# edenartlab/sd-lora-trainer

Measured on AMD Instinct MI355X. Metric: training images/sec, SDXL 1024px rank-16 LoRA, 1/2/4/8 GPU (job-parallel), higher is better.
Workload: dtype bf16

## Files before the change

### include/sdlt_kernels.h

```cpp
#ifndef SDLT_KERNELS_H
#define SDLT_KERNELS_H
#include <stdint.h>
#ifdef __cplusplus
extern "C" {
#endif

const char* sdlt_last_error(void);
int sdlt_abi_version(void);
int sdlt_struct_size(int which);

typedef struct sdlt_gemm_batch_item {
  const void* X; const void* W;
  const void* Adown; const void* Bup; void* T_out;
  void* C; void* Ct;
  const float* bias;
  const float* col_scale;
} sdlt_gemm_batch_item;

typedef struct sdlt_gemm_params {
  const void* X; int64_t ldx;
  const void* W; int64_t ldw;
  int32_t M, N, K;
  const void* X2; int64_t ldx2;
  const void* W2; int64_t ldw2;
// ... 58 lines not shown
  const void* Q; int64_t ldq;
  float* out;
  int32_t M, Cw, R, Rp;
  int32_t rank_major;
  int32_t accumulate;
  int32_t conv, Hin, Win, Cin, Hout, Wout, stride;
  const void* zero;
  int32_t first_block;
  int32_t pad_;
} sdlt_lora_grad_desc;
int sdlt_lora_grad_grouped(const sdlt_lora_grad_desc* descs_dev, const int32_t* block_desc_dev,
                           int32_t n_blocks, int32_t Rp, int32_t mfma, void* stream);
int32_t sdlt_lora_grad_block_cols(void);
int sdlt_lora_grad_wide(const sdlt_lora_grad_desc* descs_dev, const int32_t* block_desc_dev,
                        int32_t n_blocks, int32_t Rp, int32_t mfma, void* stream);

typedef struct sdlt_attn_params {
  const void* Q; int64_t ldq;
  const void* K; int64_t ldk;
  const void* V; int64_t ldv;
  const void* Kt; int64_t ldkt;
  const void* Vt; int64_t ldvt;
  const void* Qt; int64_t ldqt;
  const void* dOt; int64_t lddot;
  void* O; int64_t ldo;
  float* L;
  const void* dO; int64_t lddo;
  float* D;
  void* dQ; int64_t lddq;
  void* dK; int64_t lddk;
// ... 490 lines not shown
```

### sd-lora-trainer_amd/_lib.py

```python
import ctypes as C
import os

import torch

_HERE = os.path.dirname(os.path.abspath(__file__))
LIB_PATH = os.environ.get("SDLT_KERNEL_LIB") or os.path.join(_HERE, "libsdlt_kernels.so")

i32, i64, f32, vp = C.c_int32, C.c_int64, C.c_float, C.c_void_p


class GemmParams(C.Structure):
    _fields_ = [
        ("X", vp), ("ldx", i64), ("W", vp), ("ldw", i64),
        ("M", i32), ("N", i32), ("K", i32),
        ("X2", vp), ("ldx2", i64), ("W2", vp), ("ldw2", i64),
        ("K2", i32), ("mode", i32),
        ("Hin", i32), ("Win", i32), ("Cin", i32), ("Hout", i32), ("Wout", i32),
        ("stride", i32), ("ups", i32), ("flip", i32), ("tr", i32),
        ("zero", vp),
        ("Adown", vp), ("ld_adown", i64), ("Bup", vp), ("ld_bup", i64),
        ("T_out", vp), ("ld_t", i64),
        ("lora_R", i32), ("lora_scale", f32), ("alpha", f32),
        ("bias", vp),
        ("rowbias", vp), ("ld_rowbias", i64), ("rows_per_batch", i32),
# ... 51 lines not shown
    _fields_ = [("dY", vp), ("lddy", i64), ("Y", vp), ("ldy", i64), ("bias", vp), ("mag", vp), ("scale", vp), ("gmag", vp), ("gB", vp),
                ("ws_off", i64), ("M", i32), ("N", i32), ("rank", i32), ("splits", i32), ("grad_scale", f32), ("accumulate", i32)]


class LoraGradDesc(C.Structure):
    _fields_ = [
        ("P", vp), ("ldp", i64), ("Q", vp), ("ldq", i64), ("out", vp),
        ("M", i32), ("Cw", i32), ("R", i32), ("Rp", i32),
        ("rank_major", i32), ("accumulate", i32),
        ("conv", i32), ("Hin", i32), ("Win", i32), ("Cin", i32), ("Hout", i32), ("Wout", i32), ("stride", i32),
        ("zero", vp),
        ("first_block", i32), ("pad_", i32),
    ]


class AttnParams(C.Structure):
    _fields_ = [
        ("Q", vp), ("ldq", i64), ("K", vp), ("ldk", i64), ("V", vp), ("ldv", i64),
        ("Kt", vp), ("ldkt", i64), ("Vt", vp), ("ldvt", i64), ("Qt", vp), ("ldqt", i64), ("dOt", vp), ("lddot", i64),
        ("O", vp), ("ldo", i64), ("L", vp),
        ("dO", vp), ("lddo", i64), ("D", vp),
        ("dQ", vp), ("lddq", i64), ("dK", vp), ("lddk", i64), ("dV", vp), ("lddv", i64),
        ("dK32", vp), ("dV32", vp), ("ld32", i64),
        ("B", i32), ("H", i32), ("Nq", i32), ("Nk", i32), ("Nqp", i32), ("Nkp", i32), ("d", i32),
        ("scale", f32), ("qsplit", i32), ("causal", i32), ("accumulate_dq", i32), ("accumulate_dk", i32), ("defer_splitsum", i32), ("d_ready", i32),
    ]


ATTN_ROUTES = ("FWD32", "FWD16_KS2", "FWD16", "BWD_CROSS_ROLES", "BWD_CROSS", "BWD_BOTH32", "BWD_BOTH16", "BWD_SPLIT")
ATTN_ROUTE_MASK = 0xF
# ... 132 lines not shown

class ShadowDesc(C.Structure):
    _fields_ = [("offset", i64), ("src_ld", i64), ("rows", i32), ("cols", i32), ("dst", vp), ("ld", i64), ("dstT", vp), ("ldT", i64)]


SYMBOLS = {
    "sdlt_last_error": (C.c_char_p, []),
    "sdlt_abi_version": (i32, []),
    "sdlt_struct_size": (i32, [i32]),
    "sdlt_add2d": (i32, [vp, i64, vp, i64, vp, i64, i32, i32, vp]),
    "sdlt_gemm_bf16": (i32, [C.POINTER(GemmParams), vp]),
    "sdlt_gemm_route": (i32, [C.POINTER(GemmParams), C.POINTER(GemmPlan)]),
    "sdlt_lora_grad_grouped": (i32, [vp, vp, i32, i32, i32, vp]),
    "sdlt_lora_grad_block_cols": (i32, []),
    "sdlt_lora_grad_wide": (i32, [vp, vp, i32, i32, i32, vp]),
    "sdlt_attn_fwd": (i32, [C.POINTER(AttnParams), vp]),
    "sdlt_attn_bwd": (i32, [C.POINTER(AttnParams), vp]),
    "sdlt_attn_route": (i32, [C.POINTER(AttnParams), i32]),
    "sdlt_attn_splitsum_batch": (i32, [vp, vp, vp, i32, vp]),
    "sdlt_groupnorm_ws_floats": (i32, [i32, i32, i32]),
    "sdlt_colsum_finish_batch": (i32, [vp, i32, i32, vp]),
    "sdlt_groupnorm_fwd": (i32, [C.POINTER(GroupNormParams), vp]),
    "sdlt_groupnorm_bwd": (i32, [C.POINTER(GroupNormParams), vp]),
    "sdlt_layernorm_fwd": (i32, [vp, i64, i32, i32, vp, vp, f32, vp, i64, vp, vp]),
    "sdlt_layernorm_bwd": (i32, [vp, i64, vp, i64, i32, i32, vp, vp, vp, i64, vp, i64, vp]),
    "sdlt_layernorm_bwd_y": (i32, [vp, i64, vp, i64, i32, i32, vp, vp, vp, vp, i64, vp, i64, vp, i64, vp]),
    "sdlt_ln_fold_adapters": (i32, [vp, i32, vp]),
    "sdlt_layernorm_bwd_slabs": (i32, [vp, i64, vp, i64, i32, i32, i32, vp, vp, vp, i64, vp, i64, vp]),
    "sdlt_geglu_fwd": (i32, [vp, i64, i32, i32, vp, i64, vp]),
    "sdlt_geglu_bwd": (i32, [vp, i64, vp, i64, i32, i32, vp, i64, vp]),
# ... 80 lines not shown
            "(hipcc --offload-arch=gfx950).  There is no CPU / PyTorch fallback for the training step.")
    lib = C.CDLL(LIB_PATH, mode=C.RTLD_GLOBAL)
    for name, (res, args) in SYMBOLS.items():
        try:
            fn = getattr(lib, name)
        except AttributeError as e:
            raise KernelLibraryError(f"{LIB_PATH} does not export {name}") from e
        fn.restype = res
        fn.argtypes = args
    for which, (name, size) in enumerate(struct_sizes()):
        if lib.sdlt_struct_size(which) != size:
            raise KernelLibraryError(f"struct layout mismatch for {name}: C {lib.sdlt_struct_size(which)} vs binding {size}")
    if C.sizeof(ResizeParams) != 48:
        raise KernelLibraryError(f"struct layout mismatch for ResizeParams: header 48 vs binding {C.sizeof(ResizeParams)}")
    for cls, size in ((HeatAccumParams, 152), (HeatOverlayParams, 80), (GemmPlan, 64), (SamplerDdParams, 128), (WindowParams, 64), (RegionParams, 64),
                      (GuidanceApgParams, 56), (GuidanceDynParams, 48)):
        if C.sizeof(cls) != size:
            raise KernelLibraryError(f"struct layout mismatch for {cls.__name__}: header {size} vs binding {C.sizeof(cls)}")
    _lib = lib
    return lib


def struct_sizes():
    mirrored = (GemmParams, LoraGradDesc, AttnParams, GroupNormParams, ShadowDesc, GemmBatchItem, DoraDesc, DoraWtDesc, DoraGradDesc, SplitsumDesc, StripParams,
                TaParams, LnSlabsParams, TaGroup)
    return [(c.__name__, C.sizeof(c)) for c in mirrored] + [("sdlt_affine_grad_item", 8 * 8), ("sdlt_wgrad_tr_item", 3 * 8), ("LnFoldDesc", C.sizeof(LnFoldDesc)), ("ColsumFinishDesc", C.sizeof(ColsumFinishDesc)),
                                                               ("WskGemmParams", C.sizeof(WskGemmParams)), ("MergeDesc", C.sizeof(MergeDesc)), ("SamplerParams", C.sizeof(SamplerParams)),
                                                               ("DeltaDesc", C.sizeof(DeltaDesc)), ("SamplerImgParams", C.sizeof(SamplerImgParams)),
                                                               ("SamplerMsParams", C.sizeof(SamplerMsParams)), ("SamplerSdeParams", C.sizeof(SamplerSdeParams)),
                                                               ("GuidanceParams", C.sizeof(GuidanceParams))]

# ... 6 lines not shown
```

### sd-lora-trainer_amd/csrc/capi.cpp

```cpp
#include <cstdarg>
#include <cstdio>
#include <mutex>
#include <hip/hip_runtime.h>
#include "../../include/sdlt_kernels.h"

static thread_local char g_err[512] = "";

void sdlt_set_error(const char* fmt, ...) {
  va_list ap;
  va_start(ap, fmt);
  vsnprintf(g_err, sizeof(g_err), fmt, ap);
  va_end(ap);
}

extern "C" const char* sdlt_last_error(void) { return g_err; }
extern "C" int sdlt_abi_version(void) { return 1; }

static_assert(sizeof(sdlt_resize_params) == 48, "sdlt_resize_params has no index below: its size is part of the header's text");
static_assert(sizeof(sdlt_sampler_dd_params) == 128, "sdlt_sampler_dd_params has no index below: its size is part of the header's text");
static_assert(sizeof(sdlt_window_params) == 64, "sdlt_window_params has no index below: its size is part of the header's text");
static_assert(sizeof(sdlt_region_params) == 64, "sdlt_region_params has no index below: its size is part of the header's text");
static_assert(sizeof(sdlt_guidance_apg_params) == 56, "sdlt_guidance_apg_params has no index below: its size is part of the header's text");
static_assert(sizeof(sdlt_guidance_dyn_params) == 48, "sdlt_guidance_dyn_params has no index below: its size is part of the header's text");

extern "C" int sdlt_struct_size(int which) {
  switch (which) {
    case 0: return (int)sizeof(sdlt_gemm_params);
    case 1: return (int)sizeof(sdlt_lora_grad_desc);
    case 2: return (int)sizeof(sdlt_attn_params);
    case 3: return (int)sizeof(sdlt_groupnorm_params);
    case 4: return (int)sizeof(sdlt_shadow_desc);
    case 5: return (int)sizeof(sdlt_gemm_batch_item);
    case 6: return (int)sizeof(sdlt_dora_desc);
    case 7: return (int)sizeof(sdlt_dora_wt_desc);
    case 8: return (int)sizeof(sdlt_dora_grad_desc);
    case 9: return (int)sizeof(sdlt_splitsum_desc);
    case 10: return (int)sizeof(sdlt_strip_params);
// ... 34 lines not shown
```

### sd-lora-trainer_amd/csrc/lora_grad.hip

```cpp
#include "common.h"
#include "../../include/sdlt_kernels.h"

namespace {

constexpr int BC = 64;
constexpr int BT = 32;

typedef __bf16 bf16x4_t __attribute__((ext_vector_type(4)));

__device__ __forceinline__ bf16x4_t lds_read_tr(uint32_t addr) {
  bf16x4_t v;
  asm volatile("ds_read_b64_tr_b16 %0, %1" : "=v"(v) : "v"(addr));
  return v;
}

template <int RP, bool WIDE = false>
__global__ __launch_bounds__(256) void lora_grad_mfma_kernel(const sdlt_lora_grad_desc* descs, const int32_t* block_desc) {
  constexpr int NR = RP / 16;
  constexpr int PT = BT * BC * 2;
  constexpr int QT = BT * RP * 2;
  constexpr int STG = PT + QT;
  constexpr int QI = QT / 1024;
  constexpr int LPS = 4 + QI;
  constexpr int RING = 2 * STG;
  constexpr int RED = 4 * BC * RP * 4;
  constexpr int SMEM = 4 * RING > RED ? 4 * RING : RED;
  __shared__ __attribute__((aligned(16))) char smem[SMEM];

  const sdlt_lora_grad_desc d = descs[block_desc[blockIdx.x]];
  const int r0 = WIDE ? (int)blockIdx.y * RP : 0;
  if (WIDE && r0 >= d.R) return;
  const int Rn = WIDE ? (d.R - r0 < RP ? d.R - r0 : RP) : d.R;
  const int cb = blockIdx.x - d.first_block;
  const int lane = threadIdx.x & 63;
  const int wave = __builtin_amdgcn_readfirstlane(threadIdx.x >> 6);
  const int c0 = cb * BC;
  const bf16_t* P = (const bf16_t*)d.P;
  const bf16_t* Q = (const bf16_t*)d.Q + r0;
  const bf16_t* Z = (const bf16_t*)d.zero;

  int tap_dy = 0, tap_dx = 0, ci0 = c0;
// ... 84 lines not shown
  }

  __syncthreads();
  float* red = (float*)smem;
#pragma unroll
  for (int f = 0; f < 4; ++f)
#pragma unroll
    for (int r = 0; r < NR; ++r)
#pragma unroll
      for (int t = 0; t < 4; ++t) {
        const int c = f * 16 + g * 4 + t, rr = r * 16 + i;
        red[(wave * BC + c) * RP + rr] = acc[f][r][t];
      }
  __syncthreads();
  const int R = d.R;
  for (int e = threadIdx.x; e < BC * Rn; e += 256) {
    int cc, r;
    if (d.rank_major) { r = e / BC; cc = e - r * BC; } else { cc = e / Rn; r = e - cc * Rn; }
    const int col = c0 + cc;
    if (col < d.Cw) {
      float v = red[cc * RP + r] + red[(BC + cc) * RP + r] + red[(2 * BC + cc) * RP + r] + red[(3 * BC + cc) * RP + r];
      float* o = d.rank_major ? d.out + (int64_t)(r0 + r) * d.Cw + col : d.out + (int64_t)col * R + r0 + r;
      *o = d.accumulate ? *o + v : v;
    }
  }
}

template <int RP, bool WIDE = false>
__global__ __launch_bounds__(256) void lora_grad_valu_kernel(const sdlt_lora_grad_desc* descs, const int32_t* block_desc) {
  __shared__ float red[BC * (RP + 1)];
// ... 51 lines not shown
    __syncthreads();
  }
  const int R = d.R;
  for (int e = threadIdx.x; e < BC * Rn; e += 256) {
    int cc, r;
    if (d.rank_major) { r = e / BC; cc = e - r * BC; } else { cc = e / Rn; r = e - cc * Rn; }
    const int col = cb * BC + cc;
    if (col < d.Cw) {
      float v = red[cc * (RP + 1) + r];
      float* o = d.rank_major ? d.out + (int64_t)(r0 + r) * d.Cw + col : d.out + (int64_t)col * R + r0 + r;
      *o = d.accumulate ? *o + v : v;
    }
  }
}

template <int RP>
void launch(const sdlt_lora_grad_desc* descs, const int32_t* block_desc, int n_blocks, bool mfma, hipStream_t s) {
  if (mfma) hipLaunchKernelGGL(lora_grad_mfma_kernel<RP>, dim3(n_blocks), dim3(256), 0, s, descs, block_desc);
  else hipLaunchKernelGGL(lora_grad_valu_kernel<RP>, dim3(n_blocks), dim3(256), 0, s, descs, block_desc);
}

}

extern "C" int sdlt_lora_grad_wide(const sdlt_lora_grad_desc* descs_dev, const int32_t* block_desc_dev,
                                   int32_t n_blocks, int32_t Rp, int32_t mfma, void* stream) {
  if (n_blocks <= 0) SDLT_FAIL(SDLT_ERR_SHAPE, "sdlt_lora_grad_wide: n_blocks=%d", n_blocks);
  if (Rp != 128 && Rp != 192 && Rp != 256) SDLT_FAIL(SDLT_ERR_UNSUPPORTED, "sdlt_lora_grad_wide: padded rank %d (128/192/256)", Rp);
  hipStream_t s = (hipStream_t)stream;
  const dim3 grid(n_blocks, Rp / 64);
  if (mfma) hipLaunchKernelGGL((lora_grad_mfma_kernel<64, true>), grid, dim3(256), 0, s, descs_dev, block_desc_dev);
  else hipLaunchKernelGGL((lora_grad_valu_kernel<64, true>), grid, dim3(256), 0, s, descs_dev, block_desc_dev);
  SDLT_CHECK_LAUNCH();
  return SDLT_OK;
}

extern "C" int32_t sdlt_lora_grad_block_cols(void) { return BC; }

extern "C" int sdlt_lora_grad_grouped(const sdlt_lora_grad_desc* descs_dev, const int32_t* block_desc_dev,
                                      int32_t n_blocks, int32_t Rp, int32_t mfma, void* stream) {
  if (n_blocks <= 0) SDLT_FAIL(SDLT_ERR_SHAPE, "sdlt_lora_grad_grouped: n_blocks=%d", n_blocks);
  hipStream_t s = (hipStream_t)stream;
  switch (Rp) {
    case 16: launch<16>(descs_dev, block_desc_dev, n_blocks, mfma != 0, s); break;
    case 32: launch<32>(descs_dev, block_desc_dev, n_blocks, mfma != 0, s); break;
    case 64: launch<64>(descs_dev, block_desc_dev, n_blocks, mfma != 0, s); break;
    default: SDLT_FAIL(SDLT_ERR_UNSUPPORTED, "sdlt_lora_grad_grouped: padded rank %d (16/32/64)", Rp);
  }
  SDLT_CHECK_LAUNCH();
  return SDLT_OK;
}
```

### sd-lora-trainer_amd/csrc/optim.hip

```cpp
#include "common.h"
#include "../../include/sdlt_kernels.h"

namespace {

struct AdamwHyper { float lr, b1, b2, eps, wd, bc1, bc2, l1c, gs; };
__device__ __forceinline__ AdamwHyper adamw_hyper(const float* hyper) {
  return {hyper[0], hyper[1], hyper[2], hyper[3], hyper[4], hyper[5], hyper[6], hyper[7], hyper[8]};
}
template <bool L1>
__device__ __forceinline__ void adamw_update(const AdamwHyper& h, float rs2, float step, float& pi, const float g_, float& mi, float& vi) {
  const float gi = L1 ? g_ * h.gs + h.l1c * (pi > 0.f ? 1.f : (pi < 0.f ? -1.f : 0.f)) : g_ * h.gs;
  mi = h.b1 * mi + (1.f - h.b1) * gi;
  vi = h.b2 * vi + (1.f - h.b2) * gi * gi;
  pi = pi * (1.f - h.lr * h.wd) - step * mi / (sqrtf(vi) * rs2 + h.eps);
}

__global__ void adamw_kernel(float* p, const float* g, float* m, float* v, int64_t n, const float* hyper, float* l1_partial, int vec) {
  const AdamwHyper h = adamw_hyper(hyper);
  const float rs2 = rsqrtf(h.bc2), step = h.lr / h.bc1;
  float l1 = 0.f;
  auto upd = [&](float& pi, const float g_, float& mi, float& vi) {
    l1 += fabsf(pi);
    adamw_update<true>(h, rs2, step, pi, g_, mi, vi);
  };
  const int64_t n4 = vec ? n >> 2 : 0;
  for (int64_t i = blockIdx.x * (int64_t)blockDim.x + threadIdx.x; i < n4; i += (int64_t)gridDim.x * blockDim.x) {
    f32x4 pv = ((const f32x4*)p)[i], mv = ((const f32x4*)m)[i], vv = ((const f32x4*)v)[i];
    const f32x4 gv = ((const f32x4*)g)[i];
#pragma unroll
    for (int k = 0; k < 4; ++k) {
// ... 477 lines not shown
```

### sd-lora-trainer_amd/ops.py

```python
import collections
import ctypes as C
import math
import os
import weakref

import torch

from . import _lib

BF16 = torch.bfloat16
F32 = torch.float32


def _stream():
    return C.c_void_p(torch.cuda.current_stream().cuda_stream)


def _p(t):
    return C.c_void_p(t.data_ptr()) if t is not None else C.c_void_p(0)


def _ld(t):
    assert t.dim() == 2 and t.stride(1) == 1, f"need a 2-D row-major view, got {tuple(t.shape)} strides {t.stride()}"
    return t.stride(0)
# ... 738 lines not shown

    def set_accumulate(self, flag):
        v = self.descs_dev.view(-1, self._stride)[:, self._accum_off:self._accum_off + 4]
        v.copy_(torch.tensor([int(flag), 0, 0, 0], dtype=torch.uint8, device=v.device).expand_as(v))

    def run(self):
        lib = _lib.load()
        if self.Rp > 64:
            _lib.check(lib.sdlt_lora_grad_wide(_p(self.descs_dev), _p(self.block_desc_dev), self.n_blocks, self.Rp, self.mfma, _stream()),
                       "sdlt_lora_grad_wide")
            return
        _lib.check(lib.sdlt_lora_grad_grouped(_p(self.descs_dev), _p(self.block_desc_dev), self.n_blocks, self.Rp, self.mfma, _stream()),
                   "sdlt_lora_grad_grouped")


def _attn_params(Q, K, V, *, B, H, Nq, Nk, Nqp, Nkp, d, scale, causal=False):
    p = _lib.AttnParams()
    for t in (Q, K, V):
        _chk2(t)
    p.Q, p.ldq, p.K, p.ldk, p.V, p.ldv = _p(Q), _ld(Q), _p(K), _ld(K), _p(V), _ld(V)
    p.B, p.H, p.Nq, p.Nk, p.Nqp, p.Nkp, p.d = B, H, Nq, Nk, Nqp, Nkp, d
    p.scale, p.qsplit, p.causal = float(scale), 1, int(causal)
    return p


def attn_fwd(Q, K, V, Vt, O, L, *, B, H, Nq, Nk, Nqp, Nkp, d, scale, causal=False, zero_D=None):
    lib = _lib.load()
    p = _attn_params(Q, K, V, B=B, H=H, Nq=Nq, Nk=Nk, Nqp=Nqp, Nkp=Nkp, d=d, scale=scale, causal=causal)
    _chk2(O), _chk2(L, F32)
    p.O, p.ldo, p.L = _p(O), _ld(O), _p(L)
# ... 1068 lines not shown
```

### sd-lora-trainer_amd/step.py

```python
import math
import os

import torch

from .clip import T_TOKENS, TP
from .daam import TokenAttentionLoss
from .ti import TiState
from .unet import CTX_PAD, F32, Runtime, UNet

assert TP == CTX_PAD


TEXT_PAIR = os.environ.get("SDLT_TEXT_PAIR", "1") != "0"




class TextStack:

    def __init__(self, rt, encoders, pool_mode="argmax", eos_token_id=49407, concurrent=False, arena=None):
        self.rt, self.encoders, self.pool_mode, self.eos = rt, encoders, pool_mode, eos_token_id
        self.arena, self._grad_plan = arena, None
        B = rt.B
        self.ids = [torch.zeros(B, T_TOKENS, dtype=torch.int64, device=rt.device) for _ in encoders]
        self.pool_rows = torch.zeros(B, dtype=torch.int64, device=rt.device)
        self.widths = [e.D for e in encoders]
        self.concurrent = bool(concurrent) and torch.device(rt.device).type == "cuda"
        self.side = [torch.cuda.Stream(device=rt.device) for _ in encoders] if self.concurrent else []
# ... 118 lines not shown

    def step(self, grads, m, v, hyper, l1_sum):
        self.rt.ops.prodigy_step(self.params, grads, self.p0, m, v, self.s, hyper, self.state, self.acc, l1_sum)

    def group(self, lr):
        st = self.state.tolist()
        return dict(d=st[0], d0=st[1], d_max=st[2], d_numerator=st[3], d_denom=st[4], d_hat=st[5], k=int(st[6]), lr=lr,
                    betas=self.betas, use_bias_correction=True)


class TrainStep:
    def __init__(self, rt: Runtime, unet: UNet, *, latent_hw, snr_gamma=5.0, v_prediction=False, l1_penalty=0.03,
                 weight_decay=0.004, grad_accum=1, betas=(0.9, 0.999), eps=1e-8, text: TextStack = None, n_tokens=3,
                 token_attention_loss_w=3e-7, ti_weight_decay=0.0, ti_std_loss_w=0.01, optimizer="adamw", ti_optimizer="adamw",
                 prodigy_d_coef=1.0, prodigy_growth_rate=1.05, text_lora_weight_decay=1e-5, process_group=None,
                 cond_reg_w=0.0, tok_cov_reg_w=0.0, cond_target_norm=None, tok_cond_reg_w=0.0, reg_caption_ids=None, ddp_wire_dtype=None, ddp_zero1=None, ddp_force=False, ti_trainable=True):
        adam8 = optimizer == "AdamW8bit"
        if adam8:
            optimizer = "adamw"
        if optimizer not in ("adamw", "prodigy"):
            raise NotImplementedError(f"Invalid optimizer_name for unet: {optimizer}")
        if ti_optimizer not in ("adamw", "prodigy"):
            raise NotImplementedError(f"Invalid optimizer_name: '{ti_optimizer}'")
        self.rt, self.unet = rt, unet
        self.ti_trainable = bool(ti_trainable)
        self.full_ft = getattr(unet, "trainer", None) is not None
        self.group = unet.trainer if self.full_ft else unet.arena
        if self.full_ft:
            l1_penalty = 0.0
        self.pg, self.world = None, 1
        self.ddp = False
# ... 58 lines not shown
        self.tok_cond_reg_w = tok_cond_reg_w if text is not None else 0.0
        self.tok_reg_loss, self.tok_reg_norm = z(1), z(1)
        if self.tok_cond_reg_w > 0.0:
            from .unet import ArenaView, clone_plan
            assert reg_caption_ids is not None, "tok_cond_reg_w > 0 needs the token ids of the regularisation captions"
            self._reg_dora_plan = None
            text.defer_dora_mag_grad = text.arena is not None and text.arena.dora
            nreg = reg_caption_ids[0].shape[0]
            self.reg_rt = Runtime(dev, nreg, act_dtype=rt.act, ops=rt.ops)
            self.reg_arena, self._reg_grad_plan = (ArenaView(text.arena) if text.arena is not None else None), None
            self.reg_encoders = [clone_plan(e, self.reg_rt, arena=self.reg_arena) for e in text.encoders]
            self.reg_ids = [i.to(dev, torch.int64).contiguous() for i in reg_caption_ids]
            self.reg_ctx = rt.zeros(nreg * CTX_PAD, cfg["cross_dim"])
            self.reg_dctx = rt.zeros(nreg * CTX_PAD, cfg["cross_dim"])
        self._micro, self._acc, self.graphs_micro = 0, None, None
        if grad_accum > 1:
            gs = [self.group.grads] + ([self.ti.grads] if self.ti is not None else []) + ([self.te_arena.grads] if self.te_arena is not None else [])
            self._acc = [(g_, torch.zeros_like(g_)) for g_ in gs]

    def set_batch(self, latent, noise, timesteps, mask, ctx=None, pooled=None, time_ids=None, ids=None, caption_token_lists=None, caption_table=None):
        for dst, src in ((self.latent, latent), (self.noise, noise), (self.mask, mask), (self.timesteps, timesteps)):
            if src is not dst:
                dst.copy_(src)
        self.timesteps_f.copy_(timesteps)
        if self.text is None:
            self.ctx.view(self.B, CTX_PAD, -1)[:, :77].copy_(ctx)
            if self.pooled is not None:
                self.pooled.copy_(pooled)
        else:
            self._cond_cached = ctx is not None
# ... 62 lines not shown

    def _phase_unet(self):
        rt, u = self.rt, self.unet
        ops = rt.ops
        ops.add_noise_nhwc(self.latent, self.noise, self.timesteps, self.acp, self.x64, self.noisy)
        pred = u.forward(self.x64, self.timesteps_f, self.ctx, self._pooled_live, self.time_ids, B=self.B, H=self.h, W=self.w)
        scale = 1.0 / self.grad_accum
        ops.masked_mse_fwd_bwd(pred, self.noise, self.noisy, self.mask, self.timesteps, self.acp, self.sums, self.loss,
                               self.dpred64, snr_gamma=self.snr_gamma, v_prediction=self.v_pred, loss_scale=scale)
        rt.daam_grads = None
        if self.text is not None and self.ta_w > 0.0:
            self.ta.forward_backward(self.mask, self.w / self.h, self.ta_w * scale)
        rt.daam_applied = False
        u.daam_backward()
        self.dctx.zero_()
        u.backward(self.dpred64, self.dctx)
        self._pred = pred

    def _phase_text_bwd(self):
        if self.text is not None:
            P = self.pooled.shape[1] if self.pooled is not None else 0
            d_pooled = self.unet.dadd_in[:, :P] if self.rt.want_dpooled else None
            if self.cond_reg_w > 0.0:
                pe = self.ctx.view(self.B, CTX_PAD, -1)[:, 2:T_TOKENS].float()
                nrm = pe.norm(dim=-1, keepdim=True)
                val = nrm.mean()
                self.cond_norm.copy_(val.reshape(1))
                self.cond_reg_loss.copy_((self.cond_reg_w * (val - self.cond_target_norm) ** 2).reshape(1))
                coef = self.cond_reg_w / self.grad_accum * 2.0 * (val - self.cond_target_norm) / (self.B * (T_TOKENS - 2))
                dv = self.dctx.view(self.B, CTX_PAD, -1)
                dv[:, 2:T_TOKENS] += (coef * pe / nrm).to(dv.dtype)
# ... 21 lines not shown
        for e, w, g in zip(self.reg_encoders, self.text.widths, self.ti.grad_rows):
            e.backward(self.reg_dctx[:, off:off + w], None, g, accumulate=True)
            off += w
        if self.reg_arena is not None:
            if self._reg_grad_plan is None:
                self._reg_grad_plan = self.rt.ops.LoraGradPlan(self.reg_arena.problems, self.reg_arena.Rp, self.rt.device)
                self._reg_grad_plan.set_accumulate(True)
            self._reg_grad_plan.run()
            if self.text.arena.dora:
                self.text.arena.dora_mag_grad()
                if self._reg_dora_plan is None:
                    grads = [dict(g, accumulate=True) for g in self.reg_arena.dora_grads]
                    self._reg_dora_plan = self.rt.ops.DoraPlan([], [], grads, self.text.arena.rank, self.text.arena.Rp, self.rt.device)
                self._reg_dora_plan.mag_grad()

    def forward_backward(self):
        self._phase_text_fwd()
        self._phase_unet()
        self._phase_text_bwd()
        return self._pred

    def _unet_optimizer(self):
        a = self.group
        l1 = None if self.full_ft else self.l1_sum
        if self.full_ft and self.prodigy is None:
            a.adamw_step(self.hyper)
            return
        if self.prodigy is not None:
            if self.world > 1:
                a.grads.mul_(1.0 / self.world)
            self.prodigy.step(a.grads, a.m, a.v, self.hyper, l1)
        else:
            self.rt.ops.adamw_fused(a.params, a.grads, a.m, a.v, self.hyper, l1)
        a.refresh_shadows()

    def sync_gradients(self):
        if self.ddp and not getattr(self, "bucketed", False):
            import torch.distributed as dist
# ... 92 lines not shown
            e.refresh_shadows()

    def _accumulate(self, release):
        if self._acc is not None:
            for g_, a in self._acc:
                a.add_(g_)
                if release:
                    g_.copy_(a)
                    a.zero_()

    def body_micro(self):
        self.forward_backward()
        self._accumulate(False)

    def body(self):
        self.forward_backward()
        if getattr(self, "bucketed", False):
            self.flush_and_reduce()
        else:
            self._accumulate(True)
            self.sync_gradients()
        self.optimizer_step()

    def _phases(self):
        if self.ddp and self.bucketed:
            tr = self.group
            opt = [self._opt_shard_phase, self._opt_post_phase] if getattr(self, "zero1", False) else [self.optimizer_step]
            return [self.forward_backward] + [(lambda b=b: tr.flush(bucket=b)) for b in range(len(tr.buckets))] + opt
        if self.ddp:
            return [lambda: (self.forward_backward(), self._accumulate(True)), self.optimizer_step]
        if self._acc is not None:
# ... 45 lines not shown
            self.dctx.zero_()
            self.dctx.view(B, CTX_PAD, -1)[:, :T_TOKENS] = (0.2 * dp).to(self.dctx.dtype)
            text.backward(self.dctx, d_pooled, ti.grad_rows)
            ti.add_regulariser(std_loss_w=0.5)
            ti.hyper[:9] = torch.tensor([lr, b1, b2, self.eps, wd, 1.0 - b1 ** k, 1.0 - b2 ** k, 0.0, 1.0], dtype=F32)
            rt.ops.adamw_fused(ti.params, ti.grads, m, v, ti.hyper, None)
            ti.refresh_tables()
            losses.append(0.2 * float(loss) + float(ti.reg_loss))
        return losses

    def grad_norm(self):
        return self._unet_grad_norm()

    def _unet_grad_norm(self):
        a = self.group
        if not self.ddp:
            return float(a.grads.norm())
        if getattr(self, "zero1", False):
            import torch.distributed as dist
            sq = torch.zeros(1, dtype=torch.float64, device=a.grads.device)
            for b in range(len(a.buckets)):
                s0, s1 = a.shard_range(b)
                sq += a.grads[s0:s1].double().pow(2).sum()
            if a.n > a.n_mat and a.z_rank == 0:
                sq += a.grads[a.n_mat:].double().pow(2).sum()
            dist.all_reduce(sq, group=self.pg)
            return math.sqrt(float(sq)) / self.world
        return float(a.grads.norm()) / self.world

    def grad_norms(self):
# ... 163 lines not shown
```

### sd-lora-trainer_amd/unet.py

```python
import copy
import os
import math

import torch

from . import ops as _ops
from .topology import CONFIGS, TIME_DIM_MULT, lora_targets, param_shapes

BF16, F32 = torch.bfloat16, torch.float32


def _pad_to(x, m):
    return (x + m - 1) // m * m


XATTN_WGS = int(os.environ.get("SDLT_XATTN_WGS", "160"))

LORA_WIDE_MIN = int(os.environ.get("SDLT_LORA_WIDE_MIN", "128"))
LORA_MAX_RANK = 256


def padded_rank(rank):
    if rank <= 64:
        return 16 if rank <= 16 else (32 if rank <= 32 else 64)
# ... 150 lines not shown
                sh.append((e["offA"], r, K, K, e["A_s"], e["At_s"]))
            else:
                cin = e["conv_cin"]
                sh.append((e["offA"], r, K, K, e["A_s"], None))
                wu = self.Wu
                for tap in range(9):
                    sh.append((e["offA"] + tap * cin, r, cin, K, None, e["Ab_s"][:, tap * wu: tap * wu + wu]))
            sh.append((e["offB"], N, r, r, e["B_s"], None if self.dora else e["Bt_s"]))
            e["A"] = self.params[e["offA"]: e["offA"] + r * K].view(r, K)
            e["B"] = self.params[e["offB"]: e["offB"] + N * r].view(N, r)
            e["gA"] = self.grads[e["offA"]: e["offA"] + r * K].view(r, K)
            e["gB"] = self.grads[e["offB"]: e["offB"] + N * r].view(N, r)
            if self.dora:
                e["M"] = self.params[e["offM"]: e["offM"] + N]
                e["gM"] = self.grads[e["offM"]: e["offM"] + N]
        self._shadow_plan = rt.ops.ShadowPlan(sh, rt.device)
        if self.ln_items:
            for it in self.ln_items:
                it["A32"] = it["entry"]["A"]
            self._ln_plan = rt.ops.LnFoldPlan(self.ln_items, rt.device)
            self._ln_plan.run()
        if self.dora:
            self._build_dora_plan()
            self.dora_plan.refresh(init=True)

    def _build_dora_plan(self):
        layers = [dict(W=e["W"], A_s=e["A_s"], B_s=e["B_s"], B32=e["B"], mag=e["M"], scale=e["scale"], Bt=e["Bt_s"], s=self.scale) for e in self.entries]
        wts = []
        for w in self.dora_wts:
            ents = w["entries"]
# ... 6 lines not shown

    def scale_of(self, entries):
        e0 = entries[0]
        return self.dscale[e0["offS"]: e0["offS"] + sum(e["N"] for e in entries)]

    def set_scale(self, scale):
        if scale == self.scale:
            return
        self.scale = scale
        if self.dora:
            self._build_dora_plan()
            self.dora_plan.refresh()

    def refresh_shadows(self):
        self._shadow_plan.run(self.params)
        if self._ln_plan is not None:
            self._ln_plan.run()
        if self.dora:
            self.dora_plan.refresh()

    def dora_mag_grad(self):
        if not self.dora:
            return
        if self._dora_ngrads != len(self.dora_grads):
            self.dora_plan.set_grads(self.dora_grads)
            self._dora_ngrads = len(self.dora_grads)
        self.dora_plan.mag_grad()

    def load(self, lora_dict):
        for e in self.entries:
            A, B, *rest = lora_dict[e["name"]]
            if rest and self.dora:
                e["M"].copy_(rest[0].reshape(-1).to(self.rt.device, F32))
            if A.dim() == 4:
# ... 1248 lines not shown
            if getattr(self, "_dtp_plan", None) is not None:
                self._dtp_plan.run()
            rt.ops.gemm(self._b["dtp_all"], self.temb_Wt, rt.dsemb)
        if rt.want_dpooled or tr is not None:
            demb = rt.ops.map_bf16(_ops.MAP_DSILU, self._b["semb_in"], rt.dsemb, self.buf("demb", B, self.tdim))
            if cfg["addition"]:
                da1s = self.a2.backward(demb)
                da1 = rt.ops.map_bf16(_ops.MAP_DSILU, self.a1._b["y"], da1s, self.buf("da1", *da1s.shape))
                self.dadd_in = self.a1.backward(da1)
            if tr is not None:
                de1s = self.t2.backward(demb)
                self.t1.weight_grad(rt.ops.map_bf16(_ops.MAP_DSILU, self.t1._b["y"], de1s, self.buf("de1", *de1s.shape)))
        if tr is not None and not tr.defer_flush:
            tr.flush()
        self._cross_kv_backward(dctx)
        self.lora_grads()

    def lora_grads(self):
        rt = self.rt
        if self.arena is not None:
            if self._grad_plan is None:
                self._grad_plan = rt.ops.LoraGradPlan(self.arena.problems, self.arena.Rp, rt.device)
            self._grad_plan.run()
            self.arena.dora_mag_grad()

    def daam_backward(self):
        rt = self.rt
        rt.daam_applied = False
        if rt.daam_grads is None or not self.cross_attns:
            return
        if getattr(self, "_daam_plan", None) is None:
# ... 85 lines not shown
```

Baseline: 24.13.

## Fuse LoRA gradient reduction with AdamW update and bf16 shadow writes

```diff
diff --git a/include/sdlt_kernels.h b/include/sdlt_kernels.h
--- a/include/sdlt_kernels.h
+++ b/include/sdlt_kernels.h
@@ -96,6 +96,15 @@
 int32_t sdlt_lora_grad_block_cols(void);
 int sdlt_lora_grad_wide(const sdlt_lora_grad_desc* descs_dev, const int32_t* block_desc_dev,
                         int32_t n_blocks, int32_t Rp, int32_t mfma, void* stream);
+typedef struct {
+  float* p; float* m; float* v;
+  void* dst_rm; int64_t ld_rm;
+  void* dst_cm; int64_t ld_cm;
+  int32_t tcols, tstep;
+} sdlt_lora_tail_desc;
+int sdlt_lora_grad_adamw(const sdlt_lora_grad_desc* descs_dev, const sdlt_lora_tail_desc* tails_dev, const int32_t* block_desc_dev,
+                         int32_t n_blocks, int32_t Rp, const float* hyper, float* l1_part, int32_t n_extra, float* l1_sum,
+                         int32_t write_grad, void* stream);
 
 typedef struct sdlt_attn_params {
   const void* Q; int64_t ldq;
diff --git a/sd-lora-trainer_amd/_lib.py b/sd-lora-trainer_amd/_lib.py
--- a/sd-lora-trainer_amd/_lib.py
+++ b/sd-lora-trainer_amd/_lib.py
@@ -89,6 +89,10 @@
     ]
 
 
+class LoraTailDesc(C.Structure):
+    _fields_ = [("p", vp), ("m", vp), ("v", vp), ("dst_rm", vp), ("ld_rm", i64), ("dst_cm", vp), ("ld_cm", i64), ("tcols", i32), ("tstep", i32)]
+
+
 class AttnParams(C.Structure):
     _fields_ = [
         ("Q", vp), ("ldq", i64), ("K", vp), ("ldk", i64), ("V", vp), ("ldv", i64),
@@ -251,6 +255,7 @@
     "sdlt_lora_grad_grouped": (i32, [vp, vp, i32, i32, i32, vp]),
     "sdlt_lora_grad_block_cols": (i32, []),
     "sdlt_lora_grad_wide": (i32, [vp, vp, i32, i32, i32, vp]),
+    "sdlt_lora_grad_adamw": (i32, [vp, vp, vp, i32, i32, vp, vp, i32, vp, i32, vp]),
     "sdlt_attn_fwd": (i32, [C.POINTER(AttnParams), vp]),
     "sdlt_attn_bwd": (i32, [C.POINTER(AttnParams), vp]),
     "sdlt_attn_route": (i32, [C.POINTER(AttnParams), i32]),
@@ -361,7 +366,7 @@
     if C.sizeof(ResizeParams) != 48:
         raise KernelLibraryError(f"struct layout mismatch for ResizeParams: header 48 vs binding {C.sizeof(ResizeParams)}")
     for cls, size in ((HeatAccumParams, 152), (HeatOverlayParams, 80), (GemmPlan, 64), (SamplerDdParams, 128), (WindowParams, 64), (RegionParams, 64),
-                      (GuidanceApgParams, 56), (GuidanceDynParams, 48)):
+                      (GuidanceApgParams, 56), (GuidanceDynParams, 48), (LoraTailDesc, 64)):
         if C.sizeof(cls) != size:
             raise KernelLibraryError(f"struct layout mismatch for {cls.__name__}: header {size} vs binding {C.sizeof(cls)}")
     _lib = lib
diff --git a/sd-lora-trainer_amd/csrc/adamw_update.h b/sd-lora-trainer_amd/csrc/adamw_update.h
--- /dev/null
+++ b/sd-lora-trainer_amd/csrc/adamw_update.h
@@ -0,0 +1,24 @@
+#pragma once
+#include <math.h>
+
+#if defined(__HIPCC__)
+#define SDLT_HD __host__ __device__ __forceinline__
+#else
+#define SDLT_HD inline
+#endif
+
+struct AdamwHyper { float lr, b1, b2, eps, wd, bc1, bc2, l1c, gs; };
+SDLT_HD AdamwHyper adamw_hyper(const float* hyper) {
+  return {hyper[0], hyper[1], hyper[2], hyper[3], hyper[4], hyper[5], hyper[6], hyper[7], hyper[8]};
+}
+template <bool L1>
+SDLT_HD void adamw_update(const AdamwHyper& h, float rs2, float step, float& pi, const float g_, float& mi, float& vi) {
+#if defined(__clang__)
+#pragma clang fp contract(off)
+#endif
+  const float gi = L1 ? fmaf(h.gs, g_, h.l1c * (pi > 0.f ? 1.f : (pi < 0.f ? -1.f : 0.f))) : g_ * h.gs;
+  mi = fmaf(h.b1, mi, (1.f - h.b1) * gi);
+  vi = fmaf(h.b2, vi, gi * ((1.f - h.b2) * gi));
+  const float decay = fmaf(-h.lr, h.wd, 1.f);
+  pi = fmaf(decay, pi, -((step * mi) / fmaf(rs2, sqrtf(vi), h.eps)));
+}
diff --git a/sd-lora-trainer_amd/csrc/capi.cpp b/sd-lora-trainer_amd/csrc/capi.cpp
--- a/sd-lora-trainer_amd/csrc/capi.cpp
+++ b/sd-lora-trainer_amd/csrc/capi.cpp
@@ -21,6 +21,7 @@
 static_assert(sizeof(sdlt_window_params) == 64, "sdlt_window_params has no index below: its size is part of the header's text");
 static_assert(sizeof(sdlt_region_params) == 64, "sdlt_region_params has no index below: its size is part of the header's text");
 static_assert(sizeof(sdlt_guidance_apg_params) == 56, "sdlt_guidance_apg_params has no index below: its size is part of the header's text");
+static_assert(sizeof(sdlt_lora_tail_desc) == 64, "sdlt_lora_tail_desc has no index below: its size is part of the header's text");
 static_assert(sizeof(sdlt_guidance_dyn_params) == 48, "sdlt_guidance_dyn_params has no index below: its size is part of the header's text");
 
 extern "C" int sdlt_struct_size(int which) {
diff --git a/sd-lora-trainer_amd/csrc/lora_grad.hip b/sd-lora-trainer_amd/csrc/lora_grad.hip
--- a/sd-lora-trainer_amd/csrc/lora_grad.hip
+++ b/sd-lora-trainer_amd/csrc/lora_grad.hip
@@ -1,4 +1,5 @@
 #include "common.h"
+#include "adamw_update.h"
 #include "../../include/sdlt_kernels.h"
 
 namespace {
@@ -14,8 +15,15 @@
   return v;
 }
 
-template <int RP, bool WIDE = false>
-__global__ __launch_bounds__(256) void lora_grad_mfma_kernel(const sdlt_lora_grad_desc* descs, const int32_t* block_desc) {
+struct TailArgs {
+  const sdlt_lora_tail_desc* tails;
+  const float* hyper;
+  float* l1_part;
+  int write_grad;
+};
+
+template <int RP, bool WIDE = false, bool TAIL = false>
+__global__ __launch_bounds__(256) void lora_grad_mfma_kernel(const sdlt_lora_grad_desc* descs, const int32_t* block_desc, TailArgs ta) {
   constexpr int NR = RP / 16;
   constexpr int PT = BT * BC * 2;
   constexpr int QT = BT * RP * 2;
@@ -24,7 +32,10 @@
   constexpr int LPS = 4 + QI;
   constexpr int RING = 2 * STG;
   constexpr int RED = 4 * BC * RP * 4;
-  constexpr int SMEM = 4 * RING > RED ? 4 * RING : RED;
+  constexpr int BTILE = BC * RP * 2;
+  constexpr int NEED = RED + (TAIL ? BTILE + 16 : 0);
+  constexpr int SMEM = 4 * RING > NEED ? 4 * RING : NEED;
+  static_assert(!TAIL || (!WIDE && RP <= 32), "the fused tail exists for rank pads 16 / 32");
   __shared__ __attribute__((aligned(16))) char smem[SMEM];
 
   const sdlt_lora_grad_desc d = descs[block_desc[blockIdx.x]];
@@ -139,6 +150,61 @@
       }
   __syncthreads();
   const int R = d.R;
+  if constexpr (TAIL) {
+    const sdlt_lora_tail_desc t = ta.tails[block_desc[blockIdx.x]];
+    const AdamwHyper h = adamw_hyper(ta.hyper);
+    const float rs2 = rsqrtf(h.bc2), step = h.lr / h.bc1;
+    bf16_t* bt = (bf16_t*)(smem + RED);
+    float l1 = 0.f;
+    for (int e = threadIdx.x; e < BC * R; e += 256) {
+      int cc, r;
+      if (d.rank_major) { r = e / BC; cc = e - r * BC; } else { cc = e / R; r = e - cc * R; }
+      const int col = c0 + cc;
+      if (col < d.Cw) {
+        const float g = red[cc * RP + r] + red[(BC + cc) * RP + r] + red[(2 * BC + cc) * RP + r] + red[(3 * BC + cc) * RP + r];
+        const int64_t idx = d.rank_major ? (int64_t)r * d.Cw + col : (int64_t)col * R + r;
+        if (ta.write_grad) d.out[idx] = g;
+        float pi = t.p[idx], mi = t.m[idx], vi = t.v[idx];
+        l1 += fabsf(pi);
+        adamw_update<true>(h, rs2, step, pi, g, mi, vi);
+        t.p[idx] = pi; t.m[idx] = mi; t.v[idx] = vi;
+        bt[cc * RP + r] = f2bf(pi);
+      }
+    }
+    float* l1w = (float*)(smem + RED + BTILE);
+    l1 = wave_sum(l1);
+    if (lane == 0) l1w[wave] = l1;
+    __syncthreads();
+    if (threadIdx.x == 0) ta.l1_part[blockIdx.x] = (l1w[0] + l1w[1]) + (l1w[2] + l1w[3]);
+    if (t.dst_rm) {
+      const int r = threadIdx.x >> 3, ch = (threadIdx.x & 7) * 8;
+      if (r < R && c0 + ch < d.Cw) {
+        const uint32_t w0 = bt[(ch + 0) * RP + r] | ((uint32_t)bt[(ch + 1) * RP + r] << 16), w1 = bt[(ch + 2) * RP + r] | ((uint32_t)bt[(ch + 3) * RP + r] << 16);
+        const uint32_t w2 = bt[(ch + 4) * RP + r] | ((uint32_t)bt[(ch + 5) * RP + r] << 16), w3 = bt[(ch + 6) * RP + r] | ((uint32_t)bt[(ch + 7) * RP + r] << 16);
+        bf16_t* o = (bf16_t*)t.dst_rm + (int64_t)r * t.ld_rm + c0 + ch;
+        if (c0 + ch + 8 <= d.Cw && (((uintptr_t)o) & 15) == 0) {
+          *(uint4*)o = make_uint4(w0, w1, w2, w3);
+        } else {
+          for (int j = 0; j < 8 && c0 + ch + j < d.Cw; ++j) o[j] = bt[(ch + j) * RP + r];
+        }
+      }
+    }
+    if (t.dst_cm) {
+      constexpr int QN = RP / 8;
+      const int cc = threadIdx.x / QN, q = (threadIdx.x % QN) * 8;
+      const int col = c0 + cc;
+      if (cc < BC && col < d.Cw && q < R) {
+        const int blk = col / t.tcols;
+        bf16_t* o = (bf16_t*)t.dst_cm + (int64_t)(col - blk * t.tcols) * t.ld_cm + (int64_t)blk * t.tstep + q;
+        if (q + 8 <= R && (((uintptr_t)o) & 15) == 0) {
+          *(uint4*)o = *(const uint4*)&bt[cc * RP + q];
+        } else {
+          for (int j = 0; j < 8 && q + j < R; ++j) o[j] = bt[cc * RP + q + j];
+        }
+      }
+    }
+    return;
+  }
   for (int e = threadIdx.x; e < BC * Rn; e += 256) {
     int cc, r;
     if (d.rank_major) { r = e / BC; cc = e - r * BC; } else { cc = e / Rn; r = e - cc * Rn; }
@@ -220,9 +286,19 @@
   }
 }
 
+__global__ __launch_bounds__(256) void tail_l1_finish_kernel(const float* part, int n, float* l1_sum) {
+  __shared__ float w[4];
+  float a = 0.f;
+  for (int i = threadIdx.x; i < n; i += 256) a += part[i];
+  a = wave_sum(a);
+  if ((threadIdx.x & 63) == 0) w[threadIdx.x >> 6] = a;
+  __syncthreads();
+  if (threadIdx.x == 0) l1_sum[0] = (w[0] + w[1]) + (w[2] + w[3]);
+}
+
 template <int RP>
 void launch(const sdlt_lora_grad_desc* descs, const int32_t* block_desc, int n_blocks, bool mfma, hipStream_t s) {
-  if (mfma) hipLaunchKernelGGL(lora_grad_mfma_kernel<RP>, dim3(n_blocks), dim3(256), 0, s, descs, block_desc);
+  if (mfma) hipLaunchKernelGGL(lora_grad_mfma_kernel<RP>, dim3(n_blocks), dim3(256), 0, s, descs, block_desc, TailArgs{});
   else hipLaunchKernelGGL(lora_grad_valu_kernel<RP>, dim3(n_blocks), dim3(256), 0, s, descs, block_desc);
 }
 
@@ -234,13 +310,30 @@
   if (Rp != 128 && Rp != 192 && Rp != 256) SDLT_FAIL(SDLT_ERR_UNSUPPORTED, "sdlt_lora_grad_wide: padded rank %d (128/192/256)", Rp);
   hipStream_t s = (hipStream_t)stream;
   const dim3 grid(n_blocks, Rp / 64);
-  if (mfma) hipLaunchKernelGGL((lora_grad_mfma_kernel<64, true>), grid, dim3(256), 0, s, descs_dev, block_desc_dev);
+  if (mfma) hipLaunchKernelGGL((lora_grad_mfma_kernel<64, true>), grid, dim3(256), 0, s, descs_dev, block_desc_dev, TailArgs{});
   else hipLaunchKernelGGL((lora_grad_valu_kernel<64, true>), grid, dim3(256), 0, s, descs_dev, block_desc_dev);
   SDLT_CHECK_LAUNCH();
   return SDLT_OK;
 }
 
 extern "C" int32_t sdlt_lora_grad_block_cols(void) { return BC; }
+
+extern "C" int sdlt_lora_grad_adamw(const sdlt_lora_grad_desc* descs_dev, const sdlt_lora_tail_desc* tails_dev, const int32_t* block_desc_dev,
+                                    int32_t n_blocks, int32_t Rp, const float* hyper, float* l1_part, int32_t n_extra, float* l1_sum,
+                                    int32_t write_grad, void* stream) {
+  if (n_blocks <= 0 || n_extra < 0 || !descs_dev || !tails_dev || !block_desc_dev || !hyper || !l1_part)
+    SDLT_FAIL(SDLT_ERR_SHAPE, "sdlt_lora_grad_adamw: n_blocks=%d, n_extra=%d or a null buffer", n_blocks, n_extra);
+  hipStream_t s = (hipStream_t)stream;
+  const TailArgs ta{tails_dev, hyper, l1_part, write_grad};
+  switch (Rp) {
+    case 16: hipLaunchKernelGGL((lora_grad_mfma_kernel<16, false, true>), dim3(n_blocks), dim3(256), 0, s, descs_dev, block_desc_dev, ta); break;
+    case 32: hipLaunchKernelGGL((lora_grad_mfma_kernel<32, false, true>), dim3(n_blocks), dim3(256), 0, s, descs_dev, block_desc_dev, ta); break;
+    default: SDLT_FAIL(SDLT_ERR_UNSUPPORTED, "sdlt_lora_grad_adamw: padded rank %d (16/32)", Rp);
+  }
+  if (l1_sum) hipLaunchKernelGGL(tail_l1_finish_kernel, dim3(1), dim3(256), 0, s, (const float*)l1_part, n_blocks + n_extra, l1_sum);
+  SDLT_CHECK_LAUNCH();
+  return SDLT_OK;
+}
 
 extern "C" int sdlt_lora_grad_grouped(const sdlt_lora_grad_desc* descs_dev, const int32_t* block_desc_dev,
                                       int32_t n_blocks, int32_t Rp, int32_t mfma, void* stream) {
diff --git a/sd-lora-trainer_amd/csrc/optim.hip b/sd-lora-trainer_amd/csrc/optim.hip
--- a/sd-lora-trainer_amd/csrc/optim.hip
+++ b/sd-lora-trainer_amd/csrc/optim.hip
@@ -1,19 +1,9 @@
 #include "common.h"
+#include "adamw_update.h"
 #include "../../include/sdlt_kernels.h"
 
 namespace {
 
-struct AdamwHyper { float lr, b1, b2, eps, wd, bc1, bc2, l1c, gs; };
-__device__ __forceinline__ AdamwHyper adamw_hyper(const float* hyper) {
-  return {hyper[0], hyper[1], hyper[2], hyper[3], hyper[4], hyper[5], hyper[6], hyper[7], hyper[8]};
-}
-template <bool L1>
-__device__ __forceinline__ void adamw_update(const AdamwHyper& h, float rs2, float step, float& pi, const float g_, float& mi, float& vi) {
-  const float gi = L1 ? g_ * h.gs + h.l1c * (pi > 0.f ? 1.f : (pi < 0.f ? -1.f : 0.f)) : g_ * h.gs;
-  mi = h.b1 * mi + (1.f - h.b1) * gi;
-  vi = h.b2 * vi + (1.f - h.b2) * gi * gi;
-  pi = pi * (1.f - h.lr * h.wd) - step * mi / (sqrtf(vi) * rs2 + h.eps);
-}
 
 __global__ void adamw_kernel(float* p, const float* g, float* m, float* v, int64_t n, const float* hyper, float* l1_partial, int vec) {
   const AdamwHyper h = adamw_hyper(hyper);
diff --git a/sd-lora-trainer_amd/ops.py b/sd-lora-trainer_amd/ops.py
--- a/sd-lora-trainer_amd/ops.py
+++ b/sd-lora-trainer_amd/ops.py
@@ -776,6 +776,77 @@
                    "sdlt_lora_grad_grouped")
 
 
+def lora_grad_mfma_ok(pr, bc=64):
+    P, Q, cv = pr["P"], pr["Q"], pr.get("conv")
+    ok = _ld(P) % 8 == 0 and _ld(Q) % 8 == 0 and pr["Cw"] % 8 == 0 and P.data_ptr() % 16 == 0 and Q.data_ptr() % 16 == 0
+    return ok and (cv is None or cv.Cin % bc == 0)
+
+
+class LoraTailPlan:
+
+    def __init__(self, problems, Rp, params, grads, m, v, dests, shadow_entries, hyper, l1_sum, device, write_grad=True):
+        assert Rp in (16, 32), Rp
+        for t in (params, grads, m, v, hyper):
+            _chk2(t, F32)
+            assert t.is_contiguous()
+        lib = _lib.load()
+        bc = lib.sdlt_lora_grad_block_cols()
+        fused = [pr for pr in problems if lora_grad_mfma_ok(pr, bc)]
+        rest = [pr for pr in problems if not lora_grad_mfma_ok(pr, bc)]
+        assert fused, "no problem of this arena can take the MFMA gradient kernel"
+        self.n_fused, self.n_rest = len(fused), len(rest)
+        self.params, self.grads, self.m, self.v, self.hyper, self.l1_sum, self.write_grad = params, grads, m, v, hyper, l1_sum, int(bool(write_grad))
+        off_of = lambda pr: (pr["out"].data_ptr() - grads.data_ptr()) // 4
+        self.grad_plan = LoraGradPlan(fused, Rp, device)
+        assert self.grad_plan.mfma == 1
+        order = sorted(range(len(fused)), key=lambda i: -fused[i]["M"])
+        tails = (_lib.LoraTailDesc * len(fused))()
+        self.keep = []
+        for i, pi in enumerate(order):
+            pr, t = fused[pi], tails[i]
+            off, n = off_of(pr), pr["Cw"] * pr["R"]
+            assert 0 <= off and off + n <= params.numel() and pr["out"].numel() == n
+            t.p, t.m, t.v = params.data_ptr() + 4 * off, m.data_ptr() + 4 * off, v.data_ptr() + 4 * off
+            ds = dests[off]
+            rm, cm = ds.get("rm"), ds.get("cm")
+            if rm is not None:
+                _chk2(rm)
+                assert rm.shape[0] >= pr["R"] and rm.shape[1] >= pr["Cw"]
+                t.dst_rm, t.ld_rm = rm.data_ptr(), _ld(rm)
+            if cm is not None:
+                _chk2(cm)
+                tcols, tstep = ds.get("tcols", pr["Cw"]), ds.get("tstep", 0)
+                nblk = (pr["Cw"] + tcols - 1) // tcols
+                assert cm.shape[0] >= min(tcols, pr["Cw"]) and cm.shape[1] >= (nblk - 1) * tstep + pr["R"]
+                t.dst_cm, t.ld_cm, t.tcols, t.tstep = cm.data_ptr(), _ld(cm), tcols, tstep
+            self.keep += [rm, cm]
+        self.tails_dev = _to_dev(tails, device)
+        self.rest_plan = LoraGradPlan(rest, Rp, device) if rest else None
+        spans = sorted((off_of(pr), off_of(pr) + pr["Cw"] * pr["R"]) for pr in rest)
+        self.ranges = []
+        for a, b in spans:
+            if self.ranges and self.ranges[-1][1] == a:
+                self.ranges[-1][1] = b
+            else:
+                self.ranges.append([a, b])
+        sh = [e for e in shadow_entries if any(a <= e[0] < b for a, b in self.ranges)]
+        self.rest_shadow = ShadowPlan(sh, device) if sh else None
+        self.l1_part = torch.zeros(self.grad_plan.n_blocks + len(self.ranges), dtype=F32, device=device)
+
+    def run(self):
+        lib = _lib.load()
+        g = self.grad_plan
+        if self.rest_plan is not None:
+            self.rest_plan.run()
+            for k, (a, b) in enumerate(self.ranges):
+                adamw_fused(self.params[a:b], self.grads[a:b], self.m[a:b], self.v[a:b], self.hyper,
+                            self.l1_part[g.n_blocks + k: g.n_blocks + k + 1] if self.l1_sum is not None else None)
+            if self.rest_shadow is not None:
+                self.rest_shadow.run(self.params)
+        _lib.check(lib.sdlt_lora_grad_adamw(_p(g.descs_dev), _p(self.tails_dev), _p(g.block_desc_dev), g.n_blocks, g.Rp, _p(self.hyper), _p(self.l1_part),
+                                            len(self.ranges), _p(self.l1_sum), self.write_grad, _stream()), "sdlt_lora_grad_adamw")
+
+
 def _attn_params(Q, K, V, *, B, H, Nq, Nk, Nqp, Nkp, d, scale, causal=False):
     p = _lib.AttnParams()
     for t in (Q, K, V):
diff --git a/sd-lora-trainer_amd/step.py b/sd-lora-trainer_amd/step.py
--- a/sd-lora-trainer_amd/step.py
+++ b/sd-lora-trainer_amd/step.py
@@ -12,6 +12,7 @@
 
 
 TEXT_PAIR = os.environ.get("SDLT_TEXT_PAIR", "1") != "0"
+TAIL_FUSED = os.environ.get("SDLT_TAIL_FUSED", "1") != "0"
 
 
 
@@ -160,7 +161,8 @@
                  weight_decay=0.004, grad_accum=1, betas=(0.9, 0.999), eps=1e-8, text: TextStack = None, n_tokens=3,
                  token_attention_loss_w=3e-7, ti_weight_decay=0.0, ti_std_loss_w=0.01, optimizer="adamw", ti_optimizer="adamw",
                  prodigy_d_coef=1.0, prodigy_growth_rate=1.05, text_lora_weight_decay=1e-5, process_group=None,
-                 cond_reg_w=0.0, tok_cov_reg_w=0.0, cond_target_norm=None, tok_cond_reg_w=0.0, reg_caption_ids=None, ddp_wire_dtype=None, ddp_zero1=None, ddp_force=False, ti_trainable=True):
+                 cond_reg_w=0.0, tok_cov_reg_w=0.0, cond_target_norm=None, tok_cond_reg_w=0.0, reg_caption_ids=None, ddp_wire_dtype=None, ddp_zero1=None, ddp_force=False, ti_trainable=True,
+                 keep_grads=True):
         adam8 = optimizer == "AdamW8bit"
         if adam8:
             optimizer = "adamw"
@@ -249,6 +251,10 @@
             self.reg_ctx = rt.zeros(nreg * CTX_PAD, cfg["cross_dim"])
             self.reg_dctx = rt.zeros(nreg * CTX_PAD, cfg["cross_dim"])
         self._micro, self._acc, self.graphs_micro = 0, None, None
+        self.keep_grads = bool(keep_grads)
+        self._tail_ok = (TAIL_FUSED and not self.full_ft and self.prodigy is None and self.pg is None and not self.ddp and grad_accum == 1
+                         and hasattr(rt.ops, "LoraTailPlan") and self.group.Rp in (16, 32) and not self.group.dora and not self.group.wide)
+        self._tail_plan, self.tail_route = None, None if self._tail_ok else "unfused"
         if grad_accum > 1:
             gs = [self.group.grads] + ([self.ti.grads] if self.ti is not None else []) + ([self.te_arena.grads] if self.te_arena is not None else [])
             self._acc = [(g_, torch.zeros_like(g_)) for g_ in gs]
@@ -341,7 +347,11 @@
         rt.daam_applied = False
         u.daam_backward()
         self.dctx.zero_()
-        u.backward(self.dpred64, self.dctx)
+        u.defer_lora_grads = self._tail_active()
+        try:
+            u.backward(self.dpred64, self.dctx)
+        finally:
+            u.defer_lora_grads = False
         self._pred = pred
 
     def _phase_text_bwd(self):
@@ -393,14 +403,37 @@
                     self._reg_dora_plan = self.rt.ops.DoraPlan([], [], grads, self.text.arena.rank, self.text.arena.Rp, self.rt.device)
                 self._reg_dora_plan.mag_grad()
 
-    def forward_backward(self):
+    def _tail_active(self):
+        if self.tail_route is None and self.group.problems:
+            ops = self.rt.ops
+            self.tail_route = "fused" if all(ops.lora_grad_mfma_ok(pr) for pr in self.group.problems) else "unfused"
+        return self.tail_route == "fused"
+
+    def _fwd_bwd_phases(self):
         self._phase_text_fwd()
         self._phase_unet()
         self._phase_text_bwd()
+
+    def forward_backward(self):
+        self._fwd_bwd_phases()
+        if self._tail_active():
+            self.unet.lora_grads()
         return self._pred
+
+    def _unet_tail(self):
+        a = self.group
+        if self._tail_plan is None:
+            self._tail_plan = self.rt.ops.LoraTailPlan(a.problems, a.Rp, a.params, a.grads, a.m, a.v, a.tail_dests(), a._shadow_entries, self.hyper, self.l1_sum,
+                                                       self.rt.device, write_grad=self.keep_grads)
+            assert self._tail_plan.n_rest == 0
+        self._tail_plan.run()
+        a.refresh_ln_fold()
 
     def _unet_optimizer(self):
         a = self.group
+        if self._tail_active():
+            self._unet_tail()
+            return
         l1 = None if self.full_ft else self.l1_sum
         if self.full_ft and self.prodigy is None:
             a.adamw_step(self.hyper)
@@ -523,7 +556,7 @@
         self._accumulate(False)
 
     def body(self):
-        self.forward_backward()
+        self._fwd_bwd_phases() if self._tail_active() else self.forward_backward()
         if getattr(self, "bucketed", False):
             self.flush_and_reduce()
         else:
@@ -599,6 +632,9 @@
 
     def _unet_grad_norm(self):
         a = self.group
+        if self.tail_route == "fused" and not self.keep_grads:
+            raise RuntimeError("TrainStep(keep_grads=False): the fused adapter tail does not write the LoRA gradients; build the step with keep_grads=True "
+                               "(or SDLT_TAIL_FUSED=0) to read gradient norms")
         if not self.ddp:
             return float(a.grads.norm())
         if getattr(self, "zero1", False):
diff --git a/sd-lora-trainer_amd/unet.py b/sd-lora-trainer_amd/unet.py
--- a/sd-lora-trainer_amd/unet.py
+++ b/sd-lora-trainer_amd/unet.py
@@ -188,6 +188,7 @@
             if self.dora:
                 e["M"] = self.params[e["offM"]: e["offM"] + N]
                 e["gM"] = self.grads[e["offM"]: e["offM"] + N]
+        self._shadow_entries = sh
         self._shadow_plan = rt.ops.ShadowPlan(sh, rt.device)
         if self.ln_items:
             for it in self.ln_items:
@@ -224,10 +225,24 @@
 
     def refresh_shadows(self):
         self._shadow_plan.run(self.params)
+        self.refresh_ln_fold()
+        if self.dora:
+            self.dora_plan.refresh()
+
+    def refresh_ln_fold(self):
         if self._ln_plan is not None:
             self._ln_plan.run()
-        if self.dora:
-            self.dora_plan.refresh()
+
+    def tail_dests(self):
+        assert not self.dora
+        d = {}
+        for e in self.entries:
+            if e["conv_cin"] is None:
+                d[e["offA"]] = dict(rm=e["A_s"], cm=e["At_s"])
+            else:
+                d[e["offA"]] = dict(rm=e["A_s"], cm=e["Ab_s"], tcols=e["conv_cin"], tstep=self.Wu)
+            d[e["offB"]] = dict(rm=e["Bt_s"], cm=e["B_s"])
+        return d
 
     def dora_mag_grad(self):
         if not self.dora:
@@ -1506,7 +1521,8 @@
         if tr is not None and not tr.defer_flush:
             tr.flush()
         self._cross_kv_backward(dctx)
-        self.lora_grads()
+        if not getattr(self, "defer_lora_grads", False):
+            self.lora_grads()
 
     def lora_grads(self):
         rt = self.rt
```

New measurement: 24.17, median of 6. Within noise of the previous version (+0.2%).
